# zhoujoey/ORB-SLAM3-Mac

Measured on AMD Instinct MI355X. Metric: ORB extract+match frames/sec, higher is better.
Workload: dtype u8; 1 GPU; vga: synthetic 640x480 batch=1024 per GPU, 8-level pyramid, 1000 feats/frame, ORB extract + Hamming 2-NN match (Frame.cc:1146) + SearchForInitialization (ORBmatcher.cc:710) vs successor frame; pipelines=1, matchers=side by side (two contexts), frames_total=1024

## Files before the change

include/orbhip.h:

```cpp
#ifndef ORBHIP_H
#define ORBHIP_H
#include <stddef.h>
#include <stdint.h>
#ifdef __cplusplus
extern "C" {
#endif

#define ORBHIP_OK 0
#define ORBHIP_E_BADARG (-1)
#define ORBHIP_E_NODEVICE (-2)
#define ORBHIP_E_HIP (-3)
#define ORBHIP_E_CAPACITY (-4)
#define ORBHIP_E_ABORTED (-5)
#define ORBHIP_E_NOTSPD (-6)
#define ORBHIP_E_EMPTY (-7)

typedef struct {
    float x, y, size, angle, response;
    int32_t octave, class_id;
} orbhip_keypoint;

typedef struct orbhip_ctx orbhip_ctx;
typedef struct orbhip_extractor orbhip_extractor;

// ... 2 lines not shown

int orbhip_ctx_create(int device, void *stream, orbhip_ctx **out);
void orbhip_ctx_destroy(orbhip_ctx *ctx);
int orbhip_ctx_synchronize(orbhip_ctx *ctx);
int orbhip_ctx_wait_for(orbhip_ctx *ctx, orbhip_ctx *other);
int orbhip_ctx_check_status(orbhip_ctx *ctx);
void *orbhip_ctx_stream(orbhip_ctx *ctx);

int orbhip_extractor_create(orbhip_ctx *ctx, int nfeatures, float scale_factor, int nlevels,
                            int ini_th_fast, int min_th_fast, orbhip_extractor **out);
void orbhip_extractor_destroy(orbhip_extractor *ext);

int orbhip_extractor_levels(const orbhip_extractor *ext);
int orbhip_extractor_table(const orbhip_extractor *ext, int which, float *out);
int orbhip_extractor_features_per_level(const orbhip_extractor *ext, int *out);
int orbhip_extractor_umax(const orbhip_extractor *ext, int *out16);

int orbhip_extractor_reserve(orbhip_extractor *ext, int width, int height, int max_batch);
int orbhip_extractor_max_keypoints(const orbhip_extractor *ext);

int orbhip_extract_batch_device(orbhip_extractor *ext, const uint8_t *d_images, int width,
                                int height, size_t row_stride, size_t frame_stride, int batch,
                                int lap0, int lap1);
int orbhip_extractor_results(orbhip_extractor *ext, orbhip_keypoint **d_kp, uint8_t **d_desc,
                             int32_t **d_count, int32_t **d_mono_index);
int orbhip_extract_batch_host(orbhip_extractor *ext, const uint8_t *h_images, int width, int height,
                              size_t row_stride, size_t frame_stride, int batch, int lap0, int lap1,
                              orbhip_keypoint *kp_out, uint8_t *desc_out, int cap,
                              int32_t *count_out, int32_t *mono_out);
int orbhip_extract_batch_host_view(orbhip_extractor *ext, const uint8_t *h_images, int width, int height, size_t row_stride,
                                   size_t frame_stride, int batch, int lap0, int lap1, const orbhip_keypoint **kp_view,
                                   const uint8_t **desc_view, int *row_capacity, const int32_t **count_view, const int32_t **mono_view);
int orbhip_extractor_blur_kernel(const orbhip_extractor *ext, int batch);

int orbhip_extractor_last_frame(orbhip_extractor *ext, int frame, const orbhip_keypoint **d_kp, const uint8_t **d_desc,
                                const orbhip_keypoint **h_kp_view, const uint8_t **h_desc_view, int32_t *count, unsigned long long *generation);

int orbhip_extractor_level_dims(const orbhip_extractor *ext, int level, int *w, int *h);
int orbhip_extractor_get_pyramid_level(orbhip_extractor *ext, int frame, int level, int padded,
                                       uint8_t *h_out, size_t out_stride);
int orbhip_extractor_get_pyramid_padded(orbhip_extractor *ext, int frame, uint8_t *const *levels_out, const size_t *strides);
int orbhip_extractor_get_blurred_level(orbhip_extractor *ext, int frame, int level,
                                       uint8_t *h_out, size_t out_stride);
int orbhip_extractor_get_fast_candidates(orbhip_extractor *ext, int frame, int level,
                                         int32_t *xs, int32_t *ys, int32_t *scores, int cap,
                                         int32_t *n_out);
int orbhip_extractor_get_level_keypoints(orbhip_extractor *ext, int frame, int level,
                                         orbhip_keypoint *out, int cap, int32_t *n_out);

int orbhip_extractor_set_graph_mode(orbhip_extractor *ext, int enable);

#define ORBHIP_STAGE_PYRAMID 0
#define ORBHIP_STAGE_FAST_CELLS 1
#define ORBHIP_STAGE_BLUR 2
#define ORBHIP_STAGE_OCTREE 3
#define ORBHIP_STAGE_DESC 4
#define ORBHIP_STAGE_ASSEMBLE 5
#define ORBHIP_STAGE_COUNT 6
int orbhip_extractor_set_profiling(orbhip_extractor *ext, int enable);
int orbhip_extractor_stage_ms(orbhip_extractor *ext, float *ms_out );

int orbhip_descriptor_distance(const uint8_t *a32, const uint8_t *b32);

int orbhip_match_bf2nn_device(orbhip_ctx *ctx, const uint8_t *d_descA, const int32_t *d_nA,
                              size_t strideA, const uint8_t *d_descB, const int32_t *d_nB,
                              size_t strideB, int pairs, int max_n, double ratio,
// ... 409 lines not shown
```

orb-slam3-mac_amd/csrc/orb_internal.h:

```cpp
#pragma once
#include <hip/hip_runtime.h>
#include <stdint.h>
#include "../../include/orbhip.h"

#define ORB_MAX_LEVELS 16
#define ORB_EDGE 19
#define ORB_MINB 16
#define ORB_HALF_PATCH 15

struct OrbLevel {
    uint8_t *img;
    uint8_t *blur;
    size_t img_frame_stride;
    size_t blur_frame_stride;
    int w, h, img_pitch, blur_pitch;
    int ncols, nrows, wcell, hcell;
    int cell_base;
    int cell_cap;
    int quota;
    int key_base, key_cap;
    int kp_base, kp_cap;
    int n_ini;
    float hx;
    float scale;
    float size;
    const int16_t *xofs; const int16_t *xalpha; const int16_t *yofs; const int16_t *ybeta;
    const uint32_t *xchunk; const uint32_t *ytab;
    int resize_mode;
};

struct OrbParams {
    OrbLevel lv[ORB_MAX_LEVELS];
    int nlevels, batch;
    int n_cus;
    int ini_th, min_th;
    int cells_per_frame;
    int keys_per_frame;
    int kps_per_frame;
    int max_kp;
    int oct_nc;
    int rows_min_batch;
    int bm_min_batch;
    int br_blocks[ORB_MAX_LEVELS + 1];
    int bs_tiles[ORB_MAX_LEVELS + 1];
    int lap0, lap1;
    uint32_t *cell_count;
    uint32_t *cell_list;
    size_t cell_list_frame_stride;
    uint32_t *keys;
    uint16_t *node_of;
    uint32_t *lvl_kp;
#define ORB_PERM_MIN_BATCH 16
    uint16_t *lvl_perm;
    float *lvl_angle;
    uint8_t *lvl_desc;
    int32_t *lvl_count;
    int32_t *lvl_ncand;
    int32_t *status;
    orbhip_keypoint *out_kp;
    uint8_t *out_desc;
    int32_t *out_count;
// ... 69 lines not shown
```

orb-slam3-mac_amd/csrc/orb_kernels.hip:

```cpp
#include "orb_internal.h"
#include "wave_dpp.h"
#include <mutex>
#include <vector>
#include <cstdio>
#include <cstdlib>

#define WAVE 64

__device__ __forceinline__ int wave_incl_scan(int v) { return wave_scan_add_dpp(v); }

__device__ __forceinline__ int block_excl_scan256(int v, int *wsum, int *total)
{
    const int lane = threadIdx.x & (WAVE - 1), wid = threadIdx.x >> 6;
    int inc = wave_incl_scan(v);
    if (lane == WAVE - 1) wsum[wid] = inc;
    __syncthreads();
    int base = 0;
#pragma unroll
    for (int w = 0; w < 4; w++) {
        int s = wsum[w];
        if (w < wid) base += s;
    }
    *total = wsum[0] + wsum[1] + wsum[2] + wsum[3];
    __syncthreads();
// ... 75 lines not shown
            for (int r = tid >> 6; r < nrows; r += 4) {
                const uint8_t *q = inb + r * RS_MAXC + sx;
                hz[r * RS_TW + dxl] = (uint16_t)((q[0] * a0 + q[1] * a1) >> 4);
            }
        }
    }
    __syncthreads();
    {
        const int c4 = tid & 15, rg = tid >> 4;
        const int dx = dx0 + 4 * c4;
        if (dx < D.w) {
#pragma unroll
            for (int rr = 0; rr < 2; rr++) {
                const int dy = dy0 + 2 * rg + rr;
                if (dy < D.h) {
                    const int r0 = r0C[rr] - ybase, b0 = b0C[rr], b1 = b1C[rr];
                    const uint2 t0 = *reinterpret_cast<const uint2 *>(&hz[r0 * RS_TW + 4 * c4]);
                    const uint2 t1 = *reinterpret_cast<const uint2 *>(&hz[(r0 + 1) * RS_TW + 4 * c4]);
                    const int u0[4] = {(int)(t0.x & 0xFFFF), (int)(t0.x >> 16), (int)(t0.y & 0xFFFF), (int)(t0.y >> 16)};
                    const int u1[4] = {(int)(t1.x & 0xFFFF), (int)(t1.x >> 16), (int)(t1.y & 0xFFFF), (int)(t1.y >> 16)};
                    uint32_t packed = 0;
#pragma unroll
                    for (int j = 0; j < 4; j++) {
                        const int v = (((b0 * u0[j]) >> 16) + ((b1 * u1[j]) >> 16) + 2) >> 2;
                        packed |= (uint32_t)(v & 255) << (8 * j);
                    }
                    *reinterpret_cast<uint32_t *>(D.img + (size_t)frame * D.img_frame_stride + (size_t)dy * D.img_pitch + dx) = packed;
                }
            }
        }
    }
}

#define RSR 16
typedef unsigned short rs_u16x2 __attribute__((ext_vector_type(2)));
__device__ __forceinline__ uint32_t rs_hpass(uint2 q, uint32_t sel, uint32_t al)
{
    const uint32_t pq = __builtin_amdgcn_perm(q.y, q.x, sel);
    return __builtin_amdgcn_udot2(__builtin_bit_cast(rs_u16x2, pq), __builtin_bit_cast(rs_u16x2, al), 0u, false) & ~15u;
}
__device__ __forceinline__ uint32_t rs_mulhi24(uint32_t a, uint32_t b)
{
    uint32_t d;
    asm("v_mul_hi_u32_u24 %0, %1, %2" : "=v"(d) : "v"(a), "v"(b));
    return d;
}
typedef uint32_t rs_u32x3 __attribute__((ext_vector_type(3)));
typedef rs_u32x3 rs_u32x3_a4 __attribute__((aligned(4)));
template <int MODE>
__device__ __forceinline__ uint2 rs_load8(const uint8_t *src, uint32_t off, uint32_t shsel)
{
    if (MODE == 0) return *reinterpret_cast<const uint2 *>(src + off);
    const rs_u32x3 v = *reinterpret_cast<const rs_u32x3_a4 *>(src + off);
    return make_uint2(__builtin_amdgcn_perm(v.y, v.x, shsel), __builtin_amdgcn_perm(v.z, v.y, shsel));
}
template <int MODE>
__global__ __launch_bounds__(256) void k_resize_rows(OrbParams P, int level, int nbx)
{
    extern __shared__ uint4 yl[];
    const OrbLevel &D = P.lv[level];
    const OrbLevel &S = P.lv[level - 1];
    const unsigned lid = xcd_logical_id(blockIdx.x, gridDim.x);
    const unsigned frame = lid / (unsigned)nbx, bx = lid - frame * (unsigned)nbx;
    const int nch = (D.w + 3) >> 2, nb = (D.h + RSR - 1) / RSR, hlast = D.h - 1;
    const int row_lo = (int)((bx * 256) / (unsigned)nch) * RSR;
    const int row_hi = min((int)((bx * 256 + 255) / (unsigned)nch) * RSR + RSR + 1, hlast);
    for (int r = row_lo + (int)threadIdx.x; r <= row_hi; r += 256) yl[r - row_lo] = reinterpret_cast<const uint4 *>(D.ytab)[r];
    __syncthreads();
    const unsigned g = bx * 256 + threadIdx.x;
    if (g >= (unsigned)(nch * nb)) return;
    const unsigned band = g / (unsigned)nch, c = g - band * (unsigned)nch;
    const uint4 *xc = reinterpret_cast<const uint4 *>(D.xchunk) + 3 * c;
    const uint4 x0 = xc[0], x1 = xc[1];
    const uint4 x2 = xc[2];
    const uint32_t al3 = x2.x, shsel = x2.y;
    const uint32_t base = x0.x, sel0 = x0.y, sel1 = x0.z, sel2 = x0.w, sel3 = x1.x, al0 = x1.y, al1 = x1.z, al2 = x1.w;
    const uint8_t *src = S.img + (size_t)frame * S.img_frame_stride;
    uint8_t *dst = D.img + (size_t)frame * D.img_frame_stride;
    const int dy0 = band * RSR;
    const uint4 *yb = yl + (dy0 - row_lo);
    const int klast = hlast - dy0;
    const uint32_t spitch = (uint32_t)S.img_pitch;
    uint4 yt[2][4];
    uint2 qa[2][4], qb[2][4];
#pragma unroll
    for (int u = 0; u < 4; u++) {
        yt[0][u] = yb[min(u, klast)];
        qa[0][u] = rs_load8<MODE>(src, __umul24(yt[0][u].x, spitch) + base, shsel);
        qb[0][u] = rs_load8<MODE>(src, __umul24(yt[0][u].y, spitch) + base, shsel);
    }
    uint32_t doff = __umul24((uint32_t)dy0, (uint32_t)D.img_pitch) + 4 * c;
#pragma unroll
    for (int g = 0; g < RSR / 4; g++) {
        if (g + 1 < RSR / 4) {
#pragma unroll
            for (int u = 0; u < 4; u++) {
                const uint4 t = yb[min(4 * (g + 1) + u, klast)];
                yt[(g + 1) & 1][u] = t;
                qa[(g + 1) & 1][u] = rs_load8<MODE>(src, __umul24(t.x, spitch) + base, shsel);
                qb[(g + 1) & 1][u] = rs_load8<MODE>(src, __umul24(t.y, spitch) + base, shsel);
            }
        }
#pragma unroll
        for (int u = 0; u < 4; u++) {
            const int k = 4 * g + u;
            const uint4 t = yt[g & 1][u];
            const uint2 a = qa[g & 1][u], bq = qb[g & 1][u];
            const uint32_t s0 = rs_mulhi24(t.z, rs_hpass(a, sel0, al0)) + rs_mulhi24(t.w, rs_hpass(bq, sel0, al0)) + 2u;
            const uint32_t s1 = rs_mulhi24(t.z, rs_hpass(a, sel1, al1)) + rs_mulhi24(t.w, rs_hpass(bq, sel1, al1)) + 2u;
            const uint32_t s2 = rs_mulhi24(t.z, rs_hpass(a, sel2, al2)) + rs_mulhi24(t.w, rs_hpass(bq, sel2, al2)) + 2u;
            const uint32_t s3 = rs_mulhi24(t.z, rs_hpass(a, sel3, al3)) + rs_mulhi24(t.w, rs_hpass(bq, sel3, al3)) + 2u;
            const uint32_t p01 = (s0 | (s1 << 16)) >> 2, p23 = (s2 | (s3 << 16)) >> 2;
            *reinterpret_cast<uint32_t *>(dst + doff) = __builtin_amdgcn_perm(p23, p01, 0x06040200u);
            doff += k < klast ? (uint32_t)D.img_pitch : 0u;
        }
    }
}

void orb_launch_resize(const OrbParams &P, int level, hipStream_t s)
{
    const OrbLevel &D = P.lv[level];
    if (D.xchunk && P.batch >= P.rows_min_batch) {
        const int nch = (D.w + 3) >> 2, nb = (D.h + RSR - 1) / RSR, nbx = (nch * nb + 255) / 256;
        const dim3 grid((unsigned)nbx * (unsigned)P.batch);
        const size_t lds = (size_t)((256 / nch + 2) * RSR + 2) * sizeof(uint4);
        if (D.resize_mode == 1) hipLaunchKernelGGL(k_resize_rows<1>, grid, dim3(256), lds, s, P, level, nbx);
        else hipLaunchKernelGGL(k_resize_rows<0>, grid, dim3(256), lds, s, P, level, nbx);
        return;
    }
    const unsigned nblocks = (unsigned)(((D.w + RS_TW - 1) / RS_TW) * ((D.h + RS_TH - 1) / RS_TH)) * (unsigned)P.batch;
    hipLaunchKernelGGL(k_resize, dim3(nblocks), dim3(256), 0, s, P, level);
}

typedef short s16x2 __attribute__((ext_vector_type(2)));
typedef uint32_t u32_unaligned __attribute__((aligned(1)));

__device__ __forceinline__ s16x2 as_s16x2(uint32_t v) { return __builtin_bit_cast(s16x2, v); }
__device__ __forceinline__ uint32_t as_u32(s16x2 v) { return __builtin_bit_cast(uint32_t, v); }
__device__ __forceinline__ s16x2 pkmin(s16x2 a, s16x2 b) { return __builtin_elementwise_min(a, b); }
__device__ __forceinline__ s16x2 pkmax(s16x2 a, s16x2 b) { return __builtin_elementwise_max(a, b); }
__device__ __forceinline__ s16x2 pkmin3(s16x2 a, s16x2 b, s16x2 c)
{
    uint32_t r;
    asm("v_pk_minimum3_f16 %0, %1, %2, %3" : "=v"(r) : "v"(as_u32(a)), "v"(as_u32(b)), "v"(as_u32(c)));
    return as_s16x2(r);
}
__device__ __forceinline__ s16x2 pkmax3(s16x2 a, s16x2 b, s16x2 c)
{
    uint32_t r;
    asm("v_pk_maximum3_f16 %0, %1, %2, %3" : "=v"(r) : "v"(as_u32(a)), "v"(as_u32(b)), "v"(as_u32(c)));
    return as_s16x2(r);
}
__device__ __forceinline__ s16x2 pair_odd(uint32_t hi, uint32_t lo) { return as_s16x2(__builtin_amdgcn_alignbit(hi, lo, 16)); }

template <int PITCH>
__device__ __forceinline__ s16x2 fc_compass(const uint32_t *q)
{
    const s16x2 v = as_s16x2(q[0]);
// ... 1113 lines not shown
        blr_band<false>(src, dst, L.img_pitch, L.blur_pitch, w, h, 4 * c, band * BLR_R, klo, khi, k01, k23, k21, k0);
    } else {
        const int e = idx - nint * nb, band = e / nedge, ce = e - band * nedge;
        const int c = ce == 0 ? 0 : nint + ce;
        blr_band<true>(src, dst, L.img_pitch, L.blur_pitch, w, h, 4 * c, band * BLR_R, klo, khi, k01, k23, k21, k0);
    }
}

typedef int v4i __attribute__((ext_vector_type(4)));
__device__ __forceinline__ v4i bm_as_v4i(uint4 v) { v4i r; r[0] = (int)v.x; r[1] = (int)v.y; r[2] = (int)v.z; r[3] = (int)v.w; return r; }
__global__ __launch_bounds__(256) void k_blur_mfma(OrbParams P, int frame0, int nframes)
{
    const int per_frame = P.bm_cols[P.nlevels];
    const unsigned wid = xcd_logical_id(blockIdx.x, gridDim.x) * 4 + (threadIdx.x >> 6);
    const int lane = threadIdx.x & 63, m = lane & 15, g = lane >> 4;
    const int fr = (int)(wid / (unsigned)per_frame), rem = (int)(wid - (unsigned)fr * (unsigned)per_frame);
    if (fr >= nframes) return;
    int level = 0;
    for (int l = 1; l < P.nlevels; l++) if (rem >= P.bm_cols[l]) level = l;
    const OrbLevel &L = P.lv[level];
    const int w = L.w, h = L.h, spitch = L.img_pitch, dpitch = L.blur_pitch;
    const int tx = rem - P.bm_cols[level], X0 = 32 * tx;
    const uint8_t *src = L.img + (size_t)(frame0 + fr) * L.img_frame_stride;
    uint8_t *dst = L.blur + (size_t)(frame0 + fr) * L.blur_frame_stride;
    int cx = X0 - 16 + 16 * g;
    cx = cx < 0 ? 0 : cx;
    if (cx + 16 > w) cx = w - 16;
    const uint4 *th = P.bm_th + ((size_t)(P.bm_cols[level] + tx) * 2) * 64 + lane;
    const v4i B0 = bm_as_v4i(th[0]), B1 = bm_as_v4i(th[64]);
    v4i TV[4];
#pragma unroll
    for (int b = 0; b < 4; b++) TV[b] = bm_as_v4i(P.bm_tv[b * 64 + lane]);
    const int init = P.bm_init;
    const v4i c_init = {init, init, init, init}, c_init_lo = {init + 32768, init + 32768, init + 32768, init + 32768};
    const int nty = (h + 57) / 58;
    auto load_window = [&](int Y0, u32x4_unaligned (&raw)[4]) {
#pragma unroll
        for (int t = 0; t < 4; t++) {
            int ya = Y0 - 3 + 16 * t + m;
            ya = ya < 0 ? -ya : ya;
            ya = ya >= h ? 2 * h - 2 - ya : ya;
            ya = min(max(ya, 0), h - 1);
            raw[t] = *reinterpret_cast<const u32x4_unaligned *>(src + (uint32_t)(__umul24((uint32_t)ya, (uint32_t)spitch) + (uint32_t)cx));
        }
    };
    u32x4_unaligned raw[4];
    load_window(0, raw);
    for (int ty = 0; ty < nty; ty++) {
        const int Y0 = 58 * ty;
        v4i A[4];
#pragma unroll
        for (int t = 0; t < 4; t++) {
            A[t][0] = (int)(raw[t].x ^ 0x80808080u); A[t][1] = (int)(raw[t].y ^ 0x80808080u); A[t][2] = (int)(raw[t].z ^ 0x80808080u); A[t][3] = (int)(raw[t].w ^ 0x80808080u);
        }
        if (ty + 1 < nty) load_window(Y0 + 58, raw);
        v4i C1[2][4];
#pragma unroll
        for (int t = 0; t < 4; t++) {
            C1[0][t] = __builtin_amdgcn_mfma_i32_16x16x64_i8(A[t], B0, c_init, 0, 0, 0);
            C1[1][t] = __builtin_amdgcn_mfma_i32_16x16x64_i8(A[t], B1, c_init, 0, 0, 0);
        }
#pragma unroll
        for (int cb = 0; cb < 2; cb++) {
            v4i Ahi, Alo;
#pragma unroll
            for (int t = 0; t < 4; t++) {
                const uint32_t pab = __builtin_amdgcn_perm((uint32_t)C1[cb][t][1], (uint32_t)C1[cb][t][0], 0x05040100u);
// ... 298 lines not shown
```

orb-slam3-mac_amd/csrc/orbhip_api.hip:

```cpp
#include "orb_internal.h"
#include <cmath>
#include <cfloat>
#include <cstdio>
#include <cstdlib>
#include <cstring>
#include <string>
#include <vector>
#include <mutex>
#include <set>
#include <utility>

static thread_local std::string g_last_error;
extern "C" const char *orbhip_last_error(void) { return g_last_error.c_str(); }
extern "C" const char *orbhip_version(void) { return "orbhip 0.1 (gfx950)"; }

#define HIP_TRY(expr)                                                                   \
    do {                                                                                \
        hipError_t _e = (expr);                                                         \
        if (_e != hipSuccess) {                                                         \
            g_last_error = std::string(#expr) + ": " + hipGetErrorString(_e);           \
            return ORBHIP_E_HIP;                                                        \
        }                                                                               \
    } while (0)

// ... 423 lines not shown
        bool ok = !getenv("ORBHIP_BLUR_TILES");
        P.br_blocks[0] = 0;
        for (int l = 0; l < e->nlevels; l++) {
            const int w = P.lv[l].w, h = P.lv[l].h;
            if (h < BLR_R + 4 || w < 16) ok = false;
            P.br_blocks[l + 1] = P.br_blocks[l] + (((w + 3) / 4) * ((h + BLR_R - 1) / BLR_R) + 255) / 256;
        }
        if (!ok) P.br_blocks[e->nlevels] = 0;
    }
    P.cell_list_frame_stride = (size_t)cells * max_cell_cap;
    int rc;
    const size_t B = (size_t)max_batch;
    for (int l = 0; l < e->nlevels; l++) {
        OrbLevel &L = P.lv[l];
        L.img_pitch = align_up(L.w, 64); L.blur_pitch = L.img_pitch;
        L.img_frame_stride = (size_t)L.img_pitch * L.h; L.blur_frame_stride = L.img_frame_stride;
        if ((rc = dev_alloc(e, &L.img, B * L.img_frame_stride + 64))) return rc;
        if ((rc = dev_alloc(e, &L.blur, B * L.blur_frame_stride + 64))) return rc;
        if (l > 0) {
            std::vector<int16_t> xo, xa, yo, yb;
            resize_tables(P.lv[l - 1].w, L.w, true, xo, xa);
            resize_tables(P.lv[l - 1].h, L.h, false, yo, yb);
            int16_t *dxo, *dxa, *dyo, *dyb;
            if ((rc = dev_alloc(e, &dxo, xo.size()))) return rc;
            if ((rc = dev_alloc(e, &dxa, xa.size()))) return rc;
            if ((rc = dev_alloc(e, &dyo, yo.size()))) return rc;
            if ((rc = dev_alloc(e, &dyb, yb.size()))) return rc;
            HIP_TRY(hipMemcpy(dxo, xo.data(), xo.size() * 2, hipMemcpyHostToDevice));
            HIP_TRY(hipMemcpy(dxa, xa.data(), xa.size() * 2, hipMemcpyHostToDevice));
            HIP_TRY(hipMemcpy(dyo, yo.data(), yo.size() * 2, hipMemcpyHostToDevice));
            HIP_TRY(hipMemcpy(dyb, yb.data(), yb.size() * 2, hipMemcpyHostToDevice));
            L.xofs = dxo; L.xalpha = dxa; L.yofs = dyo; L.ybeta = dyb;
            const int sw = P.lv[l - 1].w, sh = P.lv[l - 1].h, nch = (L.w + 3) / 4;
            std::vector<uint32_t> xc((size_t)nch * 12, 0), yt((size_t)L.h * 4);
            bool fits = sw >= 8;
            const char *rm = getenv("ORBHIP_RESIZE_MODE");
            int mode = l > 1 || (sw % 4 == 0 && sw >= 12) ? 1 : 0;
            if (rm && atoi(rm) == 0) mode = 0;
            for (int c = 0; c < nch && fits; c++) {
                const int base = std::min((int)xo[4 * c], sw - 8);
                const int base4 = l > 1 ? (base & ~3) : std::min(base & ~3, sw - 12);
                xc[12 * c] = mode ? (uint32_t)base4 : (uint32_t)base;
                xc[12 * c + 9] = 0x03020100u + 0x01010101u * (uint32_t)(base - base4);
                for (int j = 0; j < 4; j++) {
                    const int col = std::min(4 * c + j, L.w - 1);
                    const int i0 = xo[col] - base, a0 = xa[2 * col], a1 = xa[2 * col + 1];
                    int i1 = i0 + 1;
                    if (i0 < 0 || i0 > 7 || a0 < 0 || a1 < 0) { fits = false; break; }
                    if (i1 > 7) { if (a1 != 0) { fits = false; break; } i1 = i0; }
                    xc[12 * c + 1 + j] = (uint32_t)i0 | 0x0c00u | ((uint32_t)i1 << 16) | 0x0c000000u;
                    xc[12 * c + 5 + j] = (uint32_t)a0 | ((uint32_t)a1 << 16);
                }
            }
            for (int dy = 0; dy < L.h; dy++) {
                const int r = yo[dy];
                yt[4 * dy] = (uint32_t)std::min(std::max(r, 0), sh - 1);
                yt[4 * dy + 1] = (uint32_t)std::min(std::max(r + 1, 0), sh - 1);
                if (yb[2 * dy] < 0 || yb[2 * dy + 1] < 0 || yb[2 * dy] > 2048 || yb[2 * dy + 1] > 2048) fits = false;
                yt[4 * dy + 2] = (uint32_t)yb[2 * dy] << 12;
                yt[4 * dy + 3] = (uint32_t)yb[2 * dy + 1] << 12;
            }
            L.xchunk = nullptr; L.ytab = nullptr;
            if (fits && !getenv("ORBHIP_RESIZE_TILES")) {
                uint32_t *dxc, *dyt;
                if ((rc = dev_alloc(e, &dxc, xc.size()))) return rc;
                if ((rc = dev_alloc(e, &dyt, yt.size()))) return rc;
                HIP_TRY(hipMemcpy(dxc, xc.data(), xc.size() * 4, hipMemcpyHostToDevice));
                HIP_TRY(hipMemcpy(dyt, yt.data(), yt.size() * 4, hipMemcpyHostToDevice));
                L.xchunk = dxc; L.ytab = dyt;
                L.resize_mode = mode;
            }
        }
    }
    e->d_level0 = P.lv[0].img; e->level0_pitch = P.lv[0].img_pitch; e->level0_frame_stride = P.lv[0].img_frame_stride;
    {
        const char *bm_env = getenv("ORBHIP_BLUR_MFMA");
        const bool bm_force = bm_env && atoi(bm_env) == 1, bm_off = bm_env && atoi(bm_env) == 0;
        bool ok = !bm_off && (bm_force || (size_t)width * height <= (size_t)320 * 1024) && P.br_blocks[e->nlevels] > 0;
        P.bm_min_batch = bm_force ? P.rows_min_batch : 128;
        int S = 0;
        for (int i = 0; i < 7; i++) { S += e->gauss_q8[i]; if (e->gauss_q8[i] < 0 || e->gauss_q8[i] > 63) ok = false; }
        if (255 * S > 65535) ok = false;
        P.bm_cols[0] = 0;
        for (int l = 0; l < e->nlevels; l++) {
            if (P.lv[l].w < 32 || P.lv[l].h < 8) ok = false;
            P.bm_cols[l + 1] = P.bm_cols[l] + (P.lv[l].w + 31) / 32;
        }
        auto refl = [](int x, int n) { return x < 0 ? -x : (x >= n ? 2 * n - 2 - x : x); };
        std::vector<int8_t> th((size_t)P.bm_cols[e->nlevels] * 2 * 64 * 16, 0), tv((size_t)4 * 64 * 16, 0);
        for (int l = 0; l < e->nlevels && ok; l++) {
            const int w = P.lv[l].w;
            for (int tx = 0; tx < (w + 31) / 32; tx++) {
                int cxs[4];
// ... 163 lines not shown
        HIP_TRY(hipEventDestroy(ev));
    }
    const int rc = orbhip_compute_stereo_fisheye_matches_device(left->ctx, left->P.out_kp, left->P.out_desc, left->P.out_count, left->P.out_mono,
                                                                 left->P.max_kp, right->P.out_kp, right->P.out_desc, right->P.out_count,
                                                                 right->P.out_mono, right->P.max_kp, 1, max_n, cam1_type, cam1, cam2_type, cam2, Rlr,
                                                                 tlr, level_sigma2, nlevels, d_l2r, d_r2l, d_dp, d_x, d_nm);
    if (rc) return rc;
    if (right->ctx->stream != st) {
        hipEvent_t ev;
        HIP_TRY(hipEventCreateWithFlags(&ev, hipEventDisableTiming));
        HIP_TRY(hipEventRecord(ev, st));
        HIP_TRY(hipStreamWaitEvent(right->ctx->stream, ev, 0));
        HIP_TRY(hipEventDestroy(ev));
    }
    int32_t *h = (int32_t *)orbhip_ctx_pinned_internal(left->ctx, 4 * words + 16);
    if (!h) return ORBHIP_E_HIP;
    HIP_TRY(hipMemcpyAsync(h, w, 4 * words, hipMemcpyDeviceToHost, st));
    HIP_TRY(hipStreamSynchronize(st));
    memcpy(l2r_out, h, 4 * (size_t)n_left);
    if (n_right) memcpy(r2l_out, h + max_n, 4 * (size_t)n_right);
    memcpy(depth_out, h + 2 * (size_t)max_n, 4 * (size_t)n_left);
    memcpy(x3d_out, h + 3 * (size_t)max_n, 12 * (size_t)n_left);
    if (n_matches_out) *n_matches_out = h[6 * (size_t)max_n];
    return ORBHIP_OK;
}

extern "C" int orbhip_extractor_blur_kernel(const orbhip_extractor *e, int batch)
{
    if (!e || !e->max_batch) return -1;
    const OrbParams &P = e->P;
    if (P.bm_cols[e->nlevels] > 0 && batch >= P.bm_min_batch) return 2;
    if (P.br_blocks[e->nlevels] > 0 && batch >= P.rows_min_batch) return 1;
    return 0;
}

extern "C" int orbhip_extractor_set_profiling(orbhip_extractor *e, int enable)
{
    if (!e) return ORBHIP_E_BADARG;
    if (enable && !e->ev_created) {
        for (auto &slot : e->ev) for (auto &ev : slot) HIP_TRY(hipEventCreate(&ev));
        e->ev_created = true;
    }
    e->profiling = enable != 0;
    e->ev_calls = 0;
    return ORBHIP_OK;
}

extern "C" int orbhip_extractor_stage_ms(orbhip_extractor *e, float *ms_out)
{
    if (!e || !ms_out || !e->ev_created || e->ev_calls <= 0) return ORBHIP_E_BADARG;
    const int n = std::min(e->ev_calls, ORBHIP_PROF_SLOTS);
    for (int i = 0; i < ORBHIP_STAGE_COUNT; i++) ms_out[i] = 0.f;
    for (int c = 0; c < n; c++) {
        const int slot = (e->ev_calls - 1 - c) % ORBHIP_PROF_SLOTS;
        HIP_TRY(hipEventSynchronize(e->ev[slot][ORBHIP_STAGE_COUNT]));
        for (int i = 0; i < ORBHIP_STAGE_COUNT; i++) {
            float ms = 0.f;
            HIP_TRY(hipEventElapsedTime(&ms, e->ev[slot][i], e->ev[slot][i + 1]));
            ms_out[i] += ms / n;
        }
    }
    e->ev_calls = 0;
    return ORBHIP_OK;
}

static int tune_int(const char *name, int dflt) { const char *v = getenv(name); return v ? atoi(v) : dflt; }
// ... 365 lines not shown
```

orb-slam3-mac_amd/python/orbhip.py:

```python
import ctypes as C
import os
import numpy as np

try:
    import torch
except Exception:
    torch = None

_HERE = os.path.dirname(os.path.abspath(__file__))
LIB_DIR = os.path.join(os.path.dirname(_HERE), "lib")
LIB_PATH = os.path.join(LIB_DIR, "liborbhip.so")
SYNTH_PATH = os.path.join(LIB_DIR, "libsynth.so")

if not os.path.exists(LIB_PATH):
    raise ImportError(
        "liborbhip.so not built: run `python -c 'import __graft_entry__ as g; g.build()'` "
        "(there is no CPU fallback for the HIP path)")

lib = C.CDLL(LIB_PATH)

OK, E_BADARG, E_NODEVICE, E_HIP, E_CAPACITY, E_ABORTED, E_NOTSPD, E_EMPTY = 0, -1, -2, -3, -4, -5, -6, -7
STAGES = ["pyramid", "fast_cells", "blur", "octree", "desc", "assemble"]

KP_DTYPE = np.dtype([("x", "<f4"), ("y", "<f4"), ("size", "<f4"), ("angle", "<f4"),
# ... 6 lines not shown
lib.orbhip_ctx_create.argtypes = [ci, vp, C.POINTER(vp)]
lib.orbhip_ctx_destroy.argtypes = [vp]
lib.orbhip_ctx_synchronize.argtypes = [vp]
lib.orbhip_ctx_stream.argtypes = [vp]
lib.orbhip_ctx_stream.restype = vp
lib.orbhip_extractor_create.argtypes = [vp, ci, cf, ci, ci, ci, C.POINTER(vp)]
lib.orbhip_extractor_destroy.argtypes = [vp]
lib.orbhip_extractor_levels.argtypes = [vp]
lib.orbhip_extractor_table.argtypes = [vp, ci, vp]
lib.orbhip_extractor_features_per_level.argtypes = [vp, vp]
lib.orbhip_extractor_umax.argtypes = [vp, vp]
lib.orbhip_extractor_reserve.argtypes = [vp, ci, ci, ci]
lib.orbhip_extractor_max_keypoints.argtypes = [vp]
lib.orbhip_extract_batch_device.argtypes = [vp, vp, ci, ci, sz, sz, ci, ci, ci]
lib.orbhip_extractor_results.argtypes = [vp, C.POINTER(vp), C.POINTER(vp), C.POINTER(vp), C.POINTER(vp)]
lib.orbhip_extract_batch_host.argtypes = [vp, vp, ci, ci, sz, sz, ci, ci, ci, vp, vp, ci, vp, vp]
lib.orbhip_extractor_level_dims.argtypes = [vp, ci, C.POINTER(ci), C.POINTER(ci)]
lib.orbhip_extractor_get_pyramid_level.argtypes = [vp, ci, ci, ci, vp, sz]
lib.orbhip_extractor_get_blurred_level.argtypes = [vp, ci, ci, vp, sz]
lib.orbhip_extractor_get_pyramid_padded.argtypes = [vp, ci, vp, vp]
lib.orbhip_extractor_get_fast_candidates.argtypes = [vp, ci, ci, vp, vp, vp, ci, C.POINTER(C.c_int32)]
lib.orbhip_extractor_get_level_keypoints.argtypes = [vp, ci, ci, vp, ci, C.POINTER(C.c_int32)]
lib.orbhip_extractor_set_profiling.argtypes = [vp, ci]
lib.orbhip_extractor_set_graph_mode.argtypes = [vp, ci]
lib.orbhip_extractor_stage_ms.argtypes = [vp, vp]
lib.orbhip_descriptor_distance.argtypes = [vp, vp]
lib.orbhip_match_bf2nn_device.argtypes = [vp, vp, vp, sz, vp, vp, sz, ci, ci, cd, vp, vp, vp]
lib.orbhip_search_for_initialization_device.argtypes = [vp, vp, vp, vp, vp, vp, vp, ci, ci, sz, cf, cf, cf, cf, ci, cf, ci,
                                                        vp, vp, vp]
lib.orbhip_ctx_check_status.argtypes = [vp]
lib.orbhip_ctx_wait_for.argtypes = [vp, vp]
lib.orbhip_extractor_blur_kernel.argtypes = [vp, ci]
lib.orbhip_extractor_blur_kernel.restype = ci
lib.orbhip_prev_matched_init_device.argtypes = [vp, vp, sz, ci, ci, vp]
lib.orbhip_search_by_projection_device.argtypes = [vp, vp, vp, vp, ci, vp, vp, vp, vp, ci, sz, ci, cf, cf, cf, cf, ci, ci, vp, vp]
lib.orbhip_search_local_map_device.argtypes = [vp, vp, vp, vp, ci, vp, vp, vp, vp, ci, sz, ci, cf, cf, cf, cf, ci, cf, vp, vp]


class OrbHipError(RuntimeError):
    def __init__(self, code, where):
        self.code = code
        super().__init__("%s failed: %d (%s)" % (where, code, lib.orbhip_last_error().decode()))


def _chk(rc, where):
    if rc != OK:
        raise OrbHipError(rc, where)


class Context:
    def __init__(self, device=0, stream=None):
        h = vp()
        _chk(lib.orbhip_ctx_create(device, stream, C.byref(h)), "orbhip_ctx_create")
        self.h = h

    def synchronize(self):
        _chk(lib.orbhip_ctx_synchronize(self.h), "orbhip_ctx_synchronize")

    def check_status(self):
        _chk(lib.orbhip_ctx_check_status(self.h), "orbhip_ctx_check_status")

    def wait_for(self, other):
        _chk(lib.orbhip_ctx_wait_for(self.h, other.h), "orbhip_ctx_wait_for")

    @property
    def stream(self):
# ... 12 lines not shown
        _chk(lib.orbhip_extractor_create(ctx.h, nfeatures, scale_factor, nlevels, ini_th, min_th, C.byref(h)),
             "orbhip_extractor_create")
        self.h, self.ctx, self.nlevels = h, ctx, nlevels

    def close(self):
        if self.h:
            lib.orbhip_extractor_destroy(self.h)
            self.h = None

    def table(self, which):
        out = np.zeros(self.nlevels, np.float32)
        _chk(lib.orbhip_extractor_table(self.h, which, out.ctypes.data), "orbhip_extractor_table")
        return out

    def features_per_level(self):
        out = np.zeros(self.nlevels, np.int32)
        _chk(lib.orbhip_extractor_features_per_level(self.h, out.ctypes.data), "features_per_level")
        return out

    def umax(self):
        out = np.zeros(16, np.int32)
        _chk(lib.orbhip_extractor_umax(self.h, out.ctypes.data), "umax")
        return out

    def reserve(self, w, h, batch):
        _chk(lib.orbhip_extractor_reserve(self.h, w, h, batch), "orbhip_extractor_reserve")

    @property
    def max_keypoints(self):
        return lib.orbhip_extractor_max_keypoints(self.h)

    def blur_kernel(self, batch):
        return ("k_blur", "k_blur_rows", "k_blur_mfma")[lib.orbhip_extractor_blur_kernel(self.h, int(batch))]

    def set_graph_mode(self, on):
        _chk(lib.orbhip_extractor_set_graph_mode(self.h, 1 if on else 0), "orbhip_extractor_set_graph_mode")

    def set_profiling(self, on):
        _chk(lib.orbhip_extractor_set_profiling(self.h, 1 if on else 0), "set_profiling")

    def stage_ms(self):
        out = np.zeros(len(STAGES), np.float32)
        _chk(lib.orbhip_extractor_stage_ms(self.h, out.ctypes.data), "stage_ms")
        return dict(zip(STAGES, out.tolist()))

    def extract_host(self, images, lap=(0, 1000)):
        img = np.ascontiguousarray(images, np.uint8)
        if img.ndim == 2:
            img = img[None]
        B, H, W = img.shape
        self.reserve(W, H, B)
        cap = self.max_keypoints
        kp = np.zeros((B, cap), KP_DTYPE)
        desc = np.zeros((B, cap, 32), np.uint8)
        cnt = np.zeros(B, np.int32)
        mono = np.zeros(B, np.int32)
        _chk(lib.orbhip_extract_batch_host(self.h, img.ctypes.data, W, H, W, W * H, B, lap[0], lap[1],
                                           kp.ctypes.data, desc.ctypes.data, cap, cnt.ctypes.data, mono.ctypes.data),
             "orbhip_extract_batch_host")
        return [(kp[f, :cnt[f]].copy(), desc[f, :cnt[f]].copy(), int(mono[f])) for f in range(B)]

    def extract_device(self, d_ptr, w, h, row_stride, frame_stride, batch, lap=(0, 1000)):
        _chk(lib.orbhip_extract_batch_device(self.h, d_ptr, w, h, row_stride, frame_stride, batch, lap[0], lap[1]),
             "orbhip_extract_batch_device")

    def results_device(self):
# ... 726 lines not shown
```

Before: 307,200 frames/s.

## Reuse horizontally filtered source rows across output rows in banded resize kernel

The row-resize kernel now walks a per-band step table of distinct source rows instead of loading two source rows per output row. Each source row is horizontally filtered once and reused as the top row of the next output row, so global loads and hpass work roughly halve when the scale factor is near one. The host picks the largest band height whose step count fits a fixed budget and pads each band's table. A small asm barrier is also added to keep constant vectors in registers in the blur MFMA kernel. Risks include more padding steps, a different band height, and a changed LDS footprint.

```diff
diff --git a/include/orbhip.h b/include/orbhip.h
--- a/include/orbhip.h
+++ b/include/orbhip.h
@@ -58,6 +58,8 @@
                                    size_t frame_stride, int batch, int lap0, int lap1, const orbhip_keypoint **kp_view,
                                    const uint8_t **desc_view, int *row_capacity, const int32_t **count_view, const int32_t **mono_view);
 int orbhip_extractor_blur_kernel(const orbhip_extractor *ext, int batch);
+
+int orbhip_extractor_resize_band_rows(const orbhip_extractor *ext, int level);
 
 int orbhip_extractor_last_frame(orbhip_extractor *ext, int frame, const orbhip_keypoint **d_kp, const uint8_t **d_desc,
                                 const orbhip_keypoint **h_kp_view, const uint8_t **h_desc_view, int32_t *count, unsigned long long *generation);
diff --git a/orb-slam3-mac_amd/csrc/orb_internal.h b/orb-slam3-mac_amd/csrc/orb_internal.h
--- a/orb-slam3-mac_amd/csrc/orb_internal.h
+++ b/orb-slam3-mac_amd/csrc/orb_internal.h
@@ -7,6 +7,7 @@
 #define ORB_EDGE 19
 #define ORB_MINB 16
 #define ORB_HALF_PATCH 15
+#define ORB_RS_STEPS 24
 
 struct OrbLevel {
     uint8_t *img;
@@ -27,6 +28,7 @@
     const int16_t *xofs; const int16_t *xalpha; const int16_t *yofs; const int16_t *ybeta;
     const uint32_t *xchunk; const uint32_t *ytab;
     int resize_mode;
+    int rs_rows;
 };
 
 struct OrbParams {
diff --git a/orb-slam3-mac_amd/csrc/orb_kernels.hip b/orb-slam3-mac_amd/csrc/orb_kernels.hip
--- a/orb-slam3-mac_amd/csrc/orb_kernels.hip
+++ b/orb-slam3-mac_amd/csrc/orb_kernels.hip
@@ -131,7 +131,8 @@
     }
 }
 
-#define RSR 16
+#define RS_STEPS ORB_RS_STEPS
+static_assert(RS_STEPS % 8 == 0 && RS_STEPS >= 16, "k_resize_rows prefetches its steps in groups of eight, two groups at least");
 typedef unsigned short rs_u16x2 __attribute__((ext_vector_type(2)));
 __device__ __forceinline__ uint32_t rs_hpass(uint2 q, uint32_t sel, uint32_t al)
 {
@@ -156,15 +157,14 @@
 template <int MODE>
 __global__ __launch_bounds__(256) void k_resize_rows(OrbParams P, int level, int nbx)
 {
-    extern __shared__ uint4 yl[];
+    extern __shared__ uint4 sl[];
     const OrbLevel &D = P.lv[level];
     const OrbLevel &S = P.lv[level - 1];
     const unsigned lid = xcd_logical_id(blockIdx.x, gridDim.x);
     const unsigned frame = lid / (unsigned)nbx, bx = lid - frame * (unsigned)nbx;
-    const int nch = (D.w + 3) >> 2, nb = (D.h + RSR - 1) / RSR, hlast = D.h - 1;
-    const int row_lo = (int)((bx * 256) / (unsigned)nch) * RSR;
-    const int row_hi = min((int)((bx * 256 + 255) / (unsigned)nch) * RSR + RSR + 1, hlast);
-    for (int r = row_lo + (int)threadIdx.x; r <= row_hi; r += 256) yl[r - row_lo] = reinterpret_cast<const uint4 *>(D.ytab)[r];
+    const int rsr = D.rs_rows, nch = (D.w + 3) >> 2, nb = (D.h + rsr - 1) / rsr;
+    const int band_lo = (int)((bx * 256) / (unsigned)nch), band_hi = min((int)((bx * 256 + 255) / (unsigned)nch), nb - 1);
+    for (int i = (int)threadIdx.x; i < (band_hi - band_lo + 1) * RS_STEPS; i += 256) sl[i] = reinterpret_cast<const uint4 *>(D.ytab)[band_lo * RS_STEPS + i];
     __syncthreads();
     const unsigned g = bx * 256 + threadIdx.x;
     if (g >= (unsigned)(nch * nb)) return;
@@ -176,42 +176,36 @@
     const uint32_t base = x0.x, sel0 = x0.y, sel1 = x0.z, sel2 = x0.w, sel3 = x1.x, al0 = x1.y, al1 = x1.z, al2 = x1.w;
     const uint8_t *src = S.img + (size_t)frame * S.img_frame_stride;
     uint8_t *dst = D.img + (size_t)frame * D.img_frame_stride;
-    const int dy0 = band * RSR;
-    const uint4 *yb = yl + (dy0 - row_lo);
-    const int klast = hlast - dy0;
+    const uint4 *st = sl + ((int)band - band_lo) * RS_STEPS;
     const uint32_t spitch = (uint32_t)S.img_pitch;
-    uint4 yt[2][4];
-    uint2 qa[2][4], qb[2][4];
-#pragma unroll
-    for (int u = 0; u < 4; u++) {
-        yt[0][u] = yb[min(u, klast)];
-        qa[0][u] = rs_load8<MODE>(src, __umul24(yt[0][u].x, spitch) + base, shsel);
-        qb[0][u] = rs_load8<MODE>(src, __umul24(yt[0][u].y, spitch) + base, shsel);
-    }
-    uint32_t doff = __umul24((uint32_t)dy0, (uint32_t)D.img_pitch) + 4 * c;
-#pragma unroll
-    for (int g = 0; g < RSR / 4; g++) {
-        if (g + 1 < RSR / 4) {
-#pragma unroll
-            for (int u = 0; u < 4; u++) {
-                const uint4 t = yb[min(4 * (g + 1) + u, klast)];
-                yt[(g + 1) & 1][u] = t;
-                qa[(g + 1) & 1][u] = rs_load8<MODE>(src, __umul24(t.x, spitch) + base, shsel);
-                qb[(g + 1) & 1][u] = rs_load8<MODE>(src, __umul24(t.y, spitch) + base, shsel);
-            }
-        }
-#pragma unroll
-        for (int u = 0; u < 4; u++) {
-            const int k = 4 * g + u;
-            const uint4 t = yt[g & 1][u];
-            const uint2 a = qa[g & 1][u], bq = qb[g & 1][u];
-            const uint32_t s0 = rs_mulhi24(t.z, rs_hpass(a, sel0, al0)) + rs_mulhi24(t.w, rs_hpass(bq, sel0, al0)) + 2u;
-            const uint32_t s1 = rs_mulhi24(t.z, rs_hpass(a, sel1, al1)) + rs_mulhi24(t.w, rs_hpass(bq, sel1, al1)) + 2u;
-            const uint32_t s2 = rs_mulhi24(t.z, rs_hpass(a, sel2, al2)) + rs_mulhi24(t.w, rs_hpass(bq, sel2, al2)) + 2u;
-            const uint32_t s3 = rs_mulhi24(t.z, rs_hpass(a, sel3, al3)) + rs_mulhi24(t.w, rs_hpass(bq, sel3, al3)) + 2u;
-            const uint32_t p01 = (s0 | (s1 << 16)) >> 2, p23 = (s2 | (s3 << 16)) >> 2;
-            *reinterpret_cast<uint32_t *>(dst + doff) = __builtin_amdgcn_perm(p23, p01, 0x06040200u);
-            doff += k < klast ? (uint32_t)D.img_pitch : 0u;
+    uint2 q[2][8];
+#pragma unroll
+    for (int u = 0; u < 8; u++) q[0][u] = rs_load8<MODE>(src, __umul24(st[u].x, spitch) + base, shsel);
+    uint32_t doff = __umul24(band * (uint32_t)rsr, (uint32_t)D.img_pitch) + 4 * c;
+    uint32_t h0 = 0, h1 = 0, h2 = 0, h3 = 0;
+#pragma unroll
+    for (int g = 0; g < RS_STEPS / 8; g++) {
+        if (g + 1 < RS_STEPS / 8) {
+#pragma unroll
+            for (int u = 0; u < 8; u++) q[(g + 1) & 1][u] = rs_load8<MODE>(src, __umul24(st[8 * (g + 1) + u].x, spitch) + base, shsel);
+        }
+#pragma unroll
+        for (int u = 0; u < 8; u++) {
+            const uint2 a = q[g & 1][u];
+            const uint32_t n0 = rs_hpass(a, sel0, al0), n1 = rs_hpass(a, sel1, al1), n2 = rs_hpass(a, sel2, al2), n3 = rs_hpass(a, sel3, al3);
+            if (8 * g + u > 0) {
+                const uint4 t = st[8 * g + u];
+                const uint32_t s0 = rs_mulhi24(t.z, h0) + rs_mulhi24(t.w, n0) + 2u;
+                const uint32_t s1 = rs_mulhi24(t.z, h1) + rs_mulhi24(t.w, n1) + 2u;
+                const uint32_t s2 = rs_mulhi24(t.z, h2) + rs_mulhi24(t.w, n2) + 2u;
+                const uint32_t s3 = rs_mulhi24(t.z, h3) + rs_mulhi24(t.w, n3) + 2u;
+                const uint32_t p01 = (s0 | (s1 << 16)) >> 2, p23 = (s2 | (s3 << 16)) >> 2;
+                if (t.y) {
+                    *reinterpret_cast<uint32_t *>(dst + doff) = __builtin_amdgcn_perm(p23, p01, 0x06040200u);
+                    doff += (uint32_t)D.img_pitch;
+                }
+            }
+            h0 = n0; h1 = n1; h2 = n2; h3 = n3;
         }
     }
 }
@@ -220,9 +214,9 @@
 {
     const OrbLevel &D = P.lv[level];
     if (D.xchunk && P.batch >= P.rows_min_batch) {
-        const int nch = (D.w + 3) >> 2, nb = (D.h + RSR - 1) / RSR, nbx = (nch * nb + 255) / 256;
+        const int nch = (D.w + 3) >> 2, nb = (D.h + D.rs_rows - 1) / D.rs_rows, nbx = (nch * nb + 255) / 256;
         const dim3 grid((unsigned)nbx * (unsigned)P.batch);
-        const size_t lds = (size_t)((256 / nch + 2) * RSR + 2) * sizeof(uint4);
+        const size_t lds = (size_t)((256 / nch + 2) * RS_STEPS) * sizeof(uint4);
         if (D.resize_mode == 1) hipLaunchKernelGGL(k_resize_rows<1>, grid, dim3(256), lds, s, P, level, nbx);
         else hipLaunchKernelGGL(k_resize_rows<0>, grid, dim3(256), lds, s, P, level, nbx);
         return;
@@ -1402,7 +1396,8 @@
 #pragma unroll
     for (int b = 0; b < 4; b++) TV[b] = bm_as_v4i(P.bm_tv[b * 64 + lane]);
     const int init = P.bm_init;
-    const v4i c_init = {init, init, init, init}, c_init_lo = {init + 32768, init + 32768, init + 32768, init + 32768};
+    v4i c_init = {init, init, init, init}, c_init_lo = {init + 32768, init + 32768, init + 32768, init + 32768};
+    asm volatile("" : "+v"(c_init), "+v"(c_init_lo));
     const int nty = (h + 57) / 58;
     auto load_window = [&](int Y0, u32x4_unaligned (&raw)[4]) {
 #pragma unroll
diff --git a/orb-slam3-mac_amd/csrc/orbhip_api.hip b/orb-slam3-mac_amd/csrc/orbhip_api.hip
--- a/orb-slam3-mac_amd/csrc/orbhip_api.hip
+++ b/orb-slam3-mac_amd/csrc/orbhip_api.hip
@@ -479,8 +479,8 @@
             HIP_TRY(hipMemcpy(dyb, yb.data(), yb.size() * 2, hipMemcpyHostToDevice));
             L.xofs = dxo; L.xalpha = dxa; L.yofs = dyo; L.ybeta = dyb;
             const int sw = P.lv[l - 1].w, sh = P.lv[l - 1].h, nch = (L.w + 3) / 4;
-            std::vector<uint32_t> xc((size_t)nch * 12, 0), yt((size_t)L.h * 4);
-            bool fits = sw >= 8;
+            std::vector<uint32_t> xc((size_t)nch * 12, 0), yt;
+            bool fits = sw >= 8 && nch >= 4;
             const char *rm = getenv("ORBHIP_RESIZE_MODE");
             int mode = l > 1 || (sw % 4 == 0 && sw >= 12) ? 1 : 0;
             if (rm && atoi(rm) == 0) mode = 0;
@@ -499,13 +499,35 @@
                     xc[12 * c + 5 + j] = (uint32_t)a0 | ((uint32_t)a1 << 16);
                 }
             }
-            for (int dy = 0; dy < L.h; dy++) {
-                const int r = yo[dy];
-                yt[4 * dy] = (uint32_t)std::min(std::max(r, 0), sh - 1);
-                yt[4 * dy + 1] = (uint32_t)std::min(std::max(r + 1, 0), sh - 1);
+            for (int dy = 0; dy < L.h; dy++)
                 if (yb[2 * dy] < 0 || yb[2 * dy + 1] < 0 || yb[2 * dy] > 2048 || yb[2 * dy + 1] > 2048) fits = false;
-                yt[4 * dy + 2] = (uint32_t)yb[2 * dy] << 12;
-                yt[4 * dy + 3] = (uint32_t)yb[2 * dy + 1] << 12;
+            auto band_steps = [&](int y0, int y1, std::vector<uint32_t> *out) {
+                int n = 0, prev = -1;
+                for (int dy = y0; dy < y1; dy++) {
+                    const int r0 = std::min(std::max((int)yo[dy], 0), sh - 1), r1 = std::min(std::max((int)yo[dy] + 1, 0), sh - 1);
+                    if (n == 0 || prev != r0) {
+                        if (out) { const uint32_t e[4] = {(uint32_t)r0, 0u, 0u, 0u}; out->insert(out->end(), e, e + 4); }
+                        n++;
+                    }
+                    if (out) { const uint32_t e[4] = {(uint32_t)r1, 1u, (uint32_t)yb[2 * dy] << 12, (uint32_t)yb[2 * dy + 1] << 12}; out->insert(out->end(), e, e + 4); }
+                    n++; prev = r1;
+                }
+                return n;
+            };
+            int rsr = ORB_RS_STEPS - 1;
+            for (; rsr > 1; rsr--) {
+                bool ok = true;
+                for (int y0 = 0; y0 < L.h && ok; y0 += rsr) ok = band_steps(y0, std::min(y0 + rsr, L.h), nullptr) <= ORB_RS_STEPS;
+                if (ok) break;
+            }
+            L.rs_rows = rsr;
+            for (int y0 = 0; y0 < L.h && fits; y0 += rsr) {
+                const size_t at = yt.size();
+                band_steps(y0, std::min(y0 + rsr, L.h), &yt);
+                while (yt.size() < at + 4 * ORB_RS_STEPS) {
+                    const uint32_t e[4] = {yt[yt.size() - 4], 0u, 0u, 0u};
+                    yt.insert(yt.end(), e, e + 4);
+                }
             }
             L.xchunk = nullptr; L.ytab = nullptr;
             if (fits && !getenv("ORBHIP_RESIZE_TILES")) {
@@ -735,6 +757,12 @@
     if (P.bm_cols[e->nlevels] > 0 && batch >= P.bm_min_batch) return 2;
     if (P.br_blocks[e->nlevels] > 0 && batch >= P.rows_min_batch) return 1;
     return 0;
+}
+
+extern "C" int orbhip_extractor_resize_band_rows(const orbhip_extractor *e, int level)
+{
+    if (!e || !e->max_batch || level < 1 || level >= e->nlevels) return -1;
+    return e->P.lv[level].xchunk ? e->P.lv[level].rs_rows : 0;
 }
 
 extern "C" int orbhip_extractor_set_profiling(orbhip_extractor *e, int enable)
diff --git a/orb-slam3-mac_amd/python/orbhip.py b/orb-slam3-mac_amd/python/orbhip.py
--- a/orb-slam3-mac_amd/python/orbhip.py
+++ b/orb-slam3-mac_amd/python/orbhip.py
@@ -62,6 +62,8 @@
 lib.orbhip_ctx_wait_for.argtypes = [vp, vp]
 lib.orbhip_extractor_blur_kernel.argtypes = [vp, ci]
 lib.orbhip_extractor_blur_kernel.restype = ci
+lib.orbhip_extractor_resize_band_rows.argtypes = [vp, ci]
+lib.orbhip_extractor_resize_band_rows.restype = ci
 lib.orbhip_prev_matched_init_device.argtypes = [vp, vp, sz, ci, ci, vp]
 lib.orbhip_search_by_projection_device.argtypes = [vp, vp, vp, vp, ci, vp, vp, vp, vp, ci, sz, ci, cf, cf, cf, cf, ci, ci, vp, vp]
 lib.orbhip_search_local_map_device.argtypes = [vp, vp, vp, vp, ci, vp, vp, vp, vp, ci, sz, ci, cf, cf, cf, cf, ci, cf, vp, vp]
@@ -140,6 +142,9 @@
 
     def blur_kernel(self, batch):
         return ("k_blur", "k_blur_rows", "k_blur_mfma")[lib.orbhip_extractor_blur_kernel(self.h, int(batch))]
+
+    def resize_band_rows(self, level):
+        return lib.orbhip_extractor_resize_band_rows(self.h, int(level))
 
     def set_graph_mode(self, on):
         _chk(lib.orbhip_extractor_set_graph_mode(self.h, 1 if on else 0), "orbhip_extractor_set_graph_mode")
```

Measured after the change: 315,900 frames/s, median of 6. +2.8%, better.
